# Guilucand/PanDelos

Hardware: AMD Instinct MI355X
Metric: scored gene-pairs/sec (whole node) (higher is better)
Workload: dtype u32 accumulate + f32 finalize

## Files before the change

pandelos_amd/csrc/pdl_api.hip:

```cpp
#include "pdl_common.h"

#include <algorithm>
#include <cstdlib>
#include <cstring>
#include <limits>

static thread_local std::string g_create_error = "";

#define PDL_GUARD_BEGIN try {
#define PDL_GUARD_END(ctx_)                                                       \
    } catch (const pdl_error &e) {                                                \
        if (ctx_) (ctx_)->err = e.msg; else g_create_error = e.msg;               \
        return e.code;                                                            \
    } catch (const std::bad_alloc &) {                                            \
        if (ctx_) (ctx_)->err = "host allocation failed";                         \
        return PDL_ERR_DEVICE;                                                    \
    }

template <class T> static T *xalloc(size_t n) {
    T *p = static_cast<T *>(malloc((n ? n : 1) * sizeof(T)));
    if (!p) throw std::bad_alloc();
    return p;
}

// ... 580 lines not shown
    else if (n == "join_tiny_tier2") c->opt_tiny_tier2 = value != 0;
    else if (n == "join_grid_pct") c->opt_grid_pct = (int) value;
    else if (n == "stage_timers") c->opt_stage_timers = value != 0;
    else if (n == "host_mirror") c->opt_host_mirror = value != 0;
    else if (n == "staging_cap") c->opt_staging_cap = value > 0 ? (uint64_t) value : 0;
    else if (n == "aside_test_reload") c->opt_aside_test_reload = value != 0;
    else if (n == "onepass_scan") c->opt_onepass_scan = value != 0;
    else if (n == "low_memory") c->opt_low_memory = value != 0;
    else if (n == "query_batch_bytes") {
        if (value <= 0) { c->err = "query_batch_bytes: a positive byte count"; return PDL_ERR_ARGUMENT; }
        c->opt_query_batch_bytes = (uint64_t) value;
        return PDL_OK;
    }
    else { c->err = "unknown option " + n; return PDL_ERR_ARGUMENT; }
    c->scored = false;
    return PDL_OK;
}

int pdl_dist_preprocess_begin(pdl_ctx *c, const uint8_t *d_residues, const uint64_t *d_offsets, const uint32_t *d_genome_of,
                              uint32_t n, uint64_t n_res, int k, uint32_t world, uint32_t rank, pdl_dist_slice *out) {
    if (!c || !out) return PDL_ERR_ARGUMENT;
    std::lock_guard<std::mutex> lk(c->mu);
    PDL_GUARD_BEGIN
    if (!d_offsets || !d_genome_of || (!d_residues && n_res)) PDL_FAIL(PDL_ERR_ARGUMENT, "null input pointer");
    if (((uintptr_t) d_residues & 15) != 0) PDL_FAIL(PDL_ERR_ARGUMENT, "d_residues must be 16-byte aligned");
    if (world == 0 || rank >= world || world > 64) PDL_FAIL(PDL_ERR_ARGUMENT, "rank %u of %u (at most 64 ranks)", rank, world);
    PDL_HIP(hipSetDevice(c->device));
    c->preprocessed = false; c->scored = false; c->tasks_ready = false; c->mirror_valid = false;
    c->dist = false; c->dist_stage = 0;
    adopt_device_input(c, d_residues, d_offsets, d_genome_of, n, n_res);
// ... 284 lines not shown
```

pandelos_amd/csrc/pdl_common.h:

```cpp
#pragma once

#include <atomic>
#include <chrono>

#include <hip/hip_runtime.h>

#include <cstdint>
#include <cstdio>
#include <mutex>
#include <cstdlib>
#include <string>
#include <utility>
#include <vector>

#include "../../include/pandelos_amd.h"

#define PDL_WAVE 64

#ifdef __HIPCC__
__device__ __forceinline__ void pdl_sync() {
#ifndef PDL_PLAIN_SYNCTHREADS
    asm volatile("s_waitcnt lgkmcnt(0)" ::: "memory");
#endif
    __syncthreads();
// ... 55 lines not shown
    PDL_JC_ERRORS = 6,
    PDL_JC_CURSOR_T3 = 7,
    PDL_JC_WIDE_ROWS = 9,
    PDL_JC_RELOADS = 10,
    PDL_JC_CURSOR_T0 = 11,
    PDL_JC_ROWS_T0B = 12,
    PDL_JC_CURSOR_T0B = 13,
    PDL_JC_ROWS_T1 = 14,
    PDL_JC_WORDS = 16,
};
enum : uint32_t {
    PDL_JT_CTR_WORDS = 8,
    PDL_JT_EMITTED = 8,
    PDL_JT_RELOADS = PDL_JC_RELOADS,
    PDL_JT_ROWS_T1 = 11,
    PDL_JT_WORDS = 12,
};
static_assert(PDL_JC_ROWS_T1 < PDL_JC_WORDS && PDL_JC_RELOADS < PDL_JT_WORDS && PDL_JC_CURSOR_T3 + 1 == PDL_JT_CTR_WORDS, "join counter layout");

struct pdl_error {
    int code;
    std::string msg;
};

#define PDL_HIP(expr)                                                                           \
    do {                                                                                        \
        hipError_t _e = (expr);                                                                 \
        if (_e != hipSuccess) {                                                                 \
            throw pdl_error{PDL_ERR_DEVICE, std::string(#expr) + ": " + hipGetErrorString(_e)}; \
        }                                                                                       \
    } while (0)
// ... 160 lines not shown
    DevBuf overflow_rows;
    DevBuf gene_info;
    DevBuf join_defer;
    DevBuf glb_table;
    bool glb_clean = false;
    DevBuf row_desc2;
    DevBuf mirror_cnt, mirror_ref;
    DevView taskpos_of;
    std::vector<uint32_t> h_fin;
    bool tasks_ready = false;
    DevBuf scratch2;
    DevBuf task_off;
    int cus = 0;
    uint32_t occ_tier1[5] = {0, 0, 0, 0, 0};
    uint32_t occ_tier0[2] = {0, 0}, occ_tier0b[2] = {0, 0};

    bool edges_valid = false;
    DevBuf bbh_kind, bbh_tab, e_src, e_dst, e_score;
    uint8_t *edge_mirror = nullptr;
    size_t edge_mirror_bytes = 0;
    uint64_t n_edges = 0, n_edges1 = 0;
    std::vector<uint32_t> h_bbh_at;
    std::vector<uint64_t> h_edge1, h_edge_off;

    int opt_tier1 = -1;
    int opt_tier0 = -1;
    int opt_sift_threshold = 1;
    bool opt_tiny_tier2 = false;
    bool opt_stage_timers = true;
    int opt_grid_pct = 0;
// ... 256 lines not shown
```

pandelos_amd/csrc/pdl_join.hip:

```cpp
#include "pdl_common.h"
#include "pdl_scan.h"

#include <algorithm>
#include <cstdlib>
#include <cstring>

constexpr int HBM_THREADS = 512;
constexpr uint32_t EMPTY_KEY = 0xffffffffu;
constexpr uint64_t FIELD_MASK = (1ull << 21) - 1;
constexpr uint32_t CELL_CHUNK = 16384;

struct JoinArgs {
    const uint2 *post;
    const uint4 *ranges;
    const uint2 *ranges8;
    const uint32_t *seq_off;
    const uint32_t *kseq_len;
    const uint32_t *genome_of;
    const uint4 *gene_info;
    const uint32_t *task_rows;
    const uint32_t *task_lg;
    const uint32_t *work;
    const uint4 *desc;
    uint32_t n_work;
// ... 1095 lines not shown
    desc[p] = make_uint4(p, r, e0, seq_off[r + 1] - e0);
}

struct RowCntFlag {
    const uint32_t *row_cnt; const uint32_t *mirror_cnt;
    __device__ uint32_t operator()(uint64_t p) const { return row_cnt[p] + (mirror_cnt ? mirror_cnt[p] : 0u); }
};
struct MirrorCntFlag {
    const uint32_t *mirror_cnt;
    __device__ uint32_t operator()(uint64_t p) const { return mirror_cnt[p]; }
};
struct FinOffApply {
    uint32_t *fin_off;
    __device__ void operator()(uint64_t p, uint32_t, uint32_t prefix) const { fin_off[p] = prefix; }
};
__global__ void k_gather_u32(const uint32_t *src, const uint32_t *idx, uint32_t n, uint32_t *dst, const uint32_t *ctr, const uint32_t *z64) {
    uint32_t i = blockIdx.x * blockDim.x + threadIdx.x;
    if (i < n) dst[i] = src[idx[i]];
    else if (i < n + PDL_JT_CTR_WORDS) dst[i] = ctr[i - n];
    else if (i < n + PDL_JT_EMITTED + 2) dst[i] = z64[i - n - PDL_JT_EMITTED];
    else if (i == n + PDL_JT_RELOADS) dst[i] = ctr[PDL_JC_RELOADS];
    else if (i == n + PDL_JT_ROWS_T1) dst[i] = ctr[PDL_JC_ROWS_T1];
}

struct ZeroRanges { uint4 *p[4]; unsigned long long n16[4]; };
__global__ __launch_bounds__(256) void k_zero_ranges(ZeroRanges z) {
    const unsigned long long stride = (unsigned long long) gridDim.x * 256;
#pragma unroll
    for (int r = 0; r < 4; r++)
        for (unsigned long long i = (unsigned long long) blockIdx.x * 256 + threadIdx.x; i < z.n16[r]; i += stride) z.p[r][i] = make_uint4(0, 0, 0, 0);
}

void pdl_prepare_tasks(pdl_ctx *c) {
    hipStream_t st = c->stream;
    const uint32_t N = c->N, G = c->G;
    if (!c->shard_set) { c->shard.resize(G); for (uint32_t g = 0; g < G; g++) c->shard[g] = g; }
    const uint32_t S = (uint32_t) c->shard.size();
    c->h_local_genome.assign(G, -1);
    c->h_task_row_off.assign(S + 1, 0);
    uint32_t n_rows = 0;
    for (uint32_t i = 0; i < S; i++) n_rows += c->h_genome_row_off[c->shard[i] + 1] - c->h_genome_row_off[c->shard[i]];
    const size_t words = 2 * (size_t) n_rows + N + G;
    const size_t words_all = words + S + 1;
    if (c->task_pin_words < words_all) {
// ... 109 lines not shown
    const size_t hbm_bytes = (size_t) pl.grid3 * N * ((pl.wide ? 2 : 1) * sizeof(uint64_t) + 3 * sizeof(uint32_t));
    if (c->glb_table.bytes < hbm_bytes) { c->glb_table.alloc(hbm_bytes); c->glb_clean = false; }
    if (!c->glb_clean) {
        PDL_HIP(hipMemsetAsync(c->glb_table.p, 0, hbm_bytes, c->stream));
        c->glb_clean = true;
    }
    pl.slack = 2ull * (pl.grid0 + pl.grid0b + pl.grid1 + pl.grid2 + pl.grid3) * CELL_CHUNK;
    return pl;
}

static void score_alloc_rows(pdl_ctx *c, const ScorePlan &pl) {
    const uint32_t N = c->N, G = c->G, n_rows = c->n_task_rows;
    const uint32_t S = (uint32_t) c->shard.size();
    c->MS.alloc((size_t) n_rows * G * sizeof(float) + 16);
    c->CM.alloc((size_t) S * N * sizeof(float) + 16);
    c->row_base.alloc((size_t) n_rows * 4); c->row_cnt.alloc((size_t) n_rows * 4); c->fin_off.alloc(((size_t) n_rows + 2) * 4);
    c->join_ctr.alloc(PDL_JC_WORDS * sizeof(uint32_t));
    c->row_desc.alloc((size_t) n_rows * sizeof(uint4));
    c->row_desc2.alloc((size_t) n_rows * sizeof(uint4) * (pl.tier0 ? 3 : 1));
    c->overflow_rows.alloc((size_t) n_rows * 4 * 4);
    if (pl.mirror) c->mirror_cnt.alloc((size_t) n_rows * 4 * 3 + 16);
    c->gene_info.alloc((size_t) N * sizeof(uint4));
    hipLaunchKernelGGL(k_row_desc, dim3((std::max(n_rows, N) + 255) / 256), dim3(256), 0, c->stream, c->task_rows.as<uint32_t>(), c->seq_off.as<uint32_t>(),
                       n_rows, c->row_desc.as<uint4>(), c->kseq_len.as<uint32_t>(), c->d_gen, c->taskpos_of.as<uint32_t>(), c->local_genome.as<uint32_t>(),
                       N, c->gene_info.as<uint4>());
}

static void score_alloc_cells(pdl_ctx *c, const ScorePlan &pl, unsigned long long cap, unsigned long long extra) {
    const unsigned long long fcap = pl.mirror ? 2 * cap + extra : cap;
    if (fcap >= 0xffffffffull) PDL_FAIL(PDL_ERR_UNSUPPORTED, "more than 2^32 emitted cells on one device: shard the genomes over more devices");
    DevBuf *st[5] = {&c->st_score, &c->st_perc, &c->st_tr, &c->st_col, &c->st_first};
// ... 11 lines not shown
    a.N = c->N; a.G = c->G; a.k = c->rp.k;
    a.min_kseq = (uint32_t) std::max<uint64_t>(c->min_kseq, 1); a.canonical = (c->flags & PDL_FLAG_CANONICAL_ORDER) ? 1u : 0u;
    a.MS = c->MS.as<float>(); a.CM = c->CM.as<float>();
    a.row_base = c->row_base.as<uint32_t>(); a.row_cnt = c->row_cnt.as<uint32_t>();
    a.st_score = c->st_score.as<float>(); a.st_perc = c->st_perc.as<float>(); a.st_tr = c->st_tr.as<float>();
    a.st_col = c->st_col.as<uint32_t>(); a.st_first = c->st_first.as<uint32_t>(); a.st_cap = c->st_cap;
    a.mirror = pl.mirror ? 1u : 0u;
    a.sift_threshold = c->opt_sift_threshold ? 1u : 0u;
    if (pl.mirror) {
        a.taskpos_of = c->taskpos_of.as<uint32_t>(); a.local_genome = c->local_genome.as<uint32_t>();
        a.mirror_cnt = c->mirror_cnt.as<uint32_t>();
    }
    return a;
}

static void score_join(pdl_ctx *c, const ScorePlan &pl) {
    hipStream_t st = c->stream;
    const uint32_t N = c->N, G = c->G, n_rows = c->n_task_rows;
    const uint32_t S = (uint32_t) c->shard.size();
    const int tier1 = pl.tier1;
    {
        auto n16 = [](size_t bytes) { return (unsigned long long) ((bytes + 15) / 16); };
        ZeroRanges z{};
        z.p[0] = c->MS.as<uint4>(); z.n16[0] = n16((size_t) n_rows * G * sizeof(float));
        z.p[1] = c->CM.as<uint4>(); z.n16[1] = n16((size_t) S * N * sizeof(float));
        z.p[2] = c->join_ctr.as<uint4>(); z.n16[2] = n16(PDL_JC_WORDS * sizeof(uint32_t));
        z.p[3] = pl.mirror ? c->mirror_cnt.as<uint4>() : nullptr; z.n16[3] = pl.mirror ? n16((size_t) n_rows * 4 * 3) : 0;
        const unsigned long long most = std::max(z.n16[0], z.n16[1]);
        hipLaunchKernelGGL(k_zero_ranges, dim3((uint32_t) std::min<unsigned long long>((most + 255) / 256 + 1, (unsigned long long) c->cus * 16)), dim3(256), 0, st, z);
    }
    JoinArgs a = join_args(c, pl);
    uint32_t *ctr32 = c->join_ctr.as<uint32_t>();
    uint32_t *list_a = c->overflow_rows.as<uint32_t>(), *list_b = list_a + n_rows, *list_s = list_b + n_rows, *list_s2 = list_s + n_rows;
    a.error_count = ctr32 + PDL_JC_ERRORS; a.reload_count = ctr32 + PDL_JC_RELOADS;
    a.cell_cursor = reinterpret_cast<unsigned long long *>(ctr32 + PDL_JC_CELLS);

    ev_begin(c, EV_JOIN);
    if (pl.wide) {
        hipLaunchKernelGGL(k_iota_u32, dim3((n_rows + 255) / 256), dim3(256), 0, st, list_b, n_rows);
        PDL_HIP(hipMemcpyAsync(ctr32 + PDL_JC_ROWS_T3, &c->n_task_rows, 4, hipMemcpyHostToDevice, st));
    }
    a.work = nullptr; a.desc = c->row_desc.as<uint4>(); a.n_work = pl.wide ? 0 : n_rows; a.n_work_ptr = nullptr;
    if (pl.tier0) {
        a.work_cursor = ctr32 + PDL_JC_CURSOR_T0; a.overflow_count = ctr32 + PDL_JC_ROWS_T0B; a.overflow_rows = list_s; a.work_batch = PT_BATCH;
        a.overflow_desc = c->row_desc2.as<uint4>() + n_rows;
#ifdef PDL_JOIN_PHASES
        static unsigned long long *d_phase0 = nullptr;
        if (!d_phase0) PDL_HIP(hipMalloc((void **) &d_phase0, 12 * sizeof(unsigned long long)));
        PDL_HIP(hipMemsetAsync(d_phase0, 0, 12 * sizeof(unsigned long long), st));
        a.phase = d_phase0;
#endif
        if (pl.tier0_cnt) hipLaunchKernelGGL((k_join_part<PT_T, PT_WG_PER_CU, true>), dim3(pl.grid0), dim3(PT_T), 0, st, a);
        else hipLaunchKernelGGL((k_join_part<PT_T, PT_WG_PER_CU, false>), dim3(pl.grid0), dim3(PT_T), 0, st, a);
#ifdef PDL_JOIN_PHASES
        {
            unsigned long long h[12];
            PDL_HIP(hipMemcpyAsync(h, d_phase0, sizeof(h), hipMemcpyDeviceToHost, st));
            PDL_HIP(hipStreamSynchronize(st));
            const double per = 10.0 / 1000.0 / std::max<uint32_t>(pl.grid0, 1);
            fprintf(stderr, "tier 0 phases per workgroup (us): draw + pick %.1f  stage %.1f  prefixes %.1f  walk %.1f  sift + add %.1f  finalize %.1f  | rows/wg %.1f\n",
                    h[0] * per, h[1] * per, h[2] * per, h[3] * per, h[4] * per, h[5] * per, (double) n_rows / std::max<uint32_t>(pl.grid0, 1));
            fprintf(stderr, "tier 0 counts: cycles %llu (%.2f rows, %.0f lookups each)  cycles that overflowed %llu  survivors of wave 0 %llu (x4 = %.1f %% of the lookups)  probe steps of thread 0: %llu\n",
                    h[6], (double) h[11] / std::max<unsigned long long>(h[6], 1), (double) h[10] / std::max<unsigned long long>(h[6], 1), h[7], h[8], 400.0 * h[8] / std::max<unsigned long long>(h[10], 1), h[9]);
            a.phase = nullptr;
        }
#endif
        a.desc = c->row_desc2.as<uint4>() + n_rows; a.n_work = 0; a.n_work_ptr = ctr32 + PDL_JC_ROWS_T0B;
        a.work_cursor = ctr32 + PDL_JC_CURSOR_T0B; a.overflow_count = ctr32 + PDL_JC_ROWS_T1; a.overflow_rows = list_s2; a.work_batch = 1;
        a.overflow_desc = c->row_desc2.as<uint4>() + 2 * (size_t) n_rows;
        if (pl.tier0_cnt) hipLaunchKernelGGL((k_join_part<PT_T2, PT_WGS2, true>), dim3(pl.grid0b), dim3(PT_T2), 0, st, a);
        else hipLaunchKernelGGL((k_join_part<PT_T2, PT_WGS2, false>), dim3(pl.grid0b), dim3(PT_T2), 0, st, a);
        a.desc = c->row_desc2.as<uint4>() + 2 * (size_t) n_rows; a.n_work = 0; a.n_work_ptr = ctr32 + PDL_JC_ROWS_T1;
        c->tm.join_launches += 2;
    }
    a.work_cursor = ctr32 + PDL_JC_CURSOR_T1; a.overflow_count = ctr32 + PDL_JC_ROWS_T2; a.overflow_rows = list_a; a.overflow_desc = tier1 ? c->row_desc2.as<uint4>() : nullptr;
    a.work_batch = pl.tier0 ? 1 : std::max<uint32_t>(1, std::min<uint32_t>(8, n_rows / (std::max<uint32_t>(pl.grid1, 1) * 8)));
    if (tier1 >= 9 && tier1 <= 11) {
        const unsigned long long avg = n_rows ? c->P / n_rows : 0;
        a.defer_cap = (uint32_t) std::min<unsigned long long>(std::min<unsigned long long>(std::max<unsigned long long>(4 * avg, 8192), 1u << 18), (unsigned long long) N + 64);
        a.defer_wide = (N >= (1u << 22) || pl.wide_aside) ? 1u : 0u;
        c->join_defer.alloc((size_t) pl.grid1 * a.defer_cap * (a.defer_wide ? sizeof(uint4) : sizeof(uint2)));
        a.defer = c->join_defer.p;
        static std::atomic<uint32_t> launch_serial{0};
        a.defer_serial = ++launch_serial;
    }
#ifdef PDL_JOIN_PHASES
    static unsigned long long *d_phase = nullptr;
    if (!d_phase) PDL_HIP(hipMalloc((void **) &d_phase, 10 * sizeof(unsigned long long)));
    PDL_HIP(hipMemsetAsync(d_phase, 0, 10 * sizeof(unsigned long long), st));
// ... 27 lines not shown
    a.hbm_u32 = reinterpret_cast<uint32_t *>(a.hbm_acc + (size_t) pl.grid3 * N * (pl.wide ? 2 : 1));
    a.work = list_b; a.n_work = 0; a.n_work_ptr = ctr32 + PDL_JC_ROWS_T3; a.work_cursor = ctr32 + PDL_JC_CURSOR_T3; a.work_batch = 1;
    ev_begin(c, EV_JOIN_OVF);
    c->glb_clean = false;
    if (pl.wide) hipLaunchKernelGGL(k_join_hbm<true>, dim3(pl.grid3), dim3(HBM_THREADS), 0, st, a);
    else hipLaunchKernelGGL(k_join_hbm<false>, dim3(pl.grid3), dim3(HBM_THREADS), 0, st, a);
    PDL_HIP(hipGetLastError());
    ev_end(c, EV_JOIN_OVF);
    ev_end(c, EV_JOIN);
    c->tm.join_launches += 3;
}

struct JoinCounters {
    uint32_t rows_tier2, rows_tier3, reloads;
    unsigned long long cells;
};
static JoinCounters join_counters(const uint32_t *w) {
    if (w[PDL_JC_ERRORS]) PDL_FAIL(PDL_ERR_DEVICE, "join: %u internal consistency violations", w[PDL_JC_ERRORS]);
    JoinCounters j{w[PDL_JC_ROWS_T2], w[PDL_JC_ROWS_T3], w[PDL_JC_RELOADS], 0};
    memcpy(&j.cells, w + PDL_JC_CELLS, sizeof(j.cells));
    return j;
}

static unsigned long long score_order(pdl_ctx *c, const ScorePlan &pl, const pdl_dist_cell *d_inbox, uint32_t n_inbox, int ev_total) {
    hipStream_t st = c->stream;
    const uint32_t n_rows = c->n_task_rows;
    const uint32_t S = (uint32_t) c->shard.size();
    uint64_t *d_scal = c->scalars.as<uint64_t>();
    uint32_t *ctr32 = c->join_ctr.as<uint32_t>();
    ev_begin(c, EV_ORDER);
    const uint32_t *d_mcnt = pl.mirror ? c->mirror_cnt.as<uint32_t>() : nullptr;
    scan_and_apply(c, n_rows, RowCntFlag{c->row_cnt.as<uint32_t>(), d_mcnt}, FinOffApply{c->fin_off.as<uint32_t>()}, d_scal + PDL_CTL_EMITTED,
                   reinterpret_cast<uint64_t *>(c->fin_off.as<uint32_t>() + n_rows));
    OrderArgs o{};
    if (pl.mirror) {
        uint32_t *m_off = c->mirror_cnt.as<uint32_t>() + n_rows, *m_cur = m_off + n_rows;
        scan_and_apply(c, n_rows, MirrorCntFlag{d_mcnt}, FinOffApply{m_off}, d_scal + PDL_CTL_MIRRORED);
        MirrorArgs ma{};
        ma.row_base = c->row_base.as<uint32_t>(); ma.row_cnt = c->row_cnt.as<uint32_t>(); ma.task_rows = c->task_rows.as<uint32_t>();
        ma.st_score = c->st_score.as<float>(); ma.st_perc = c->st_perc.as<float>(); ma.st_tr = c->st_tr.as<float>();
        ma.st_col = c->st_col.as<uint32_t>(); ma.st_first = c->st_first.as<uint32_t>();
        ma.taskpos_of = c->taskpos_of.as<uint32_t>(); ma.mirror_off = m_off; ma.mirror_cur = m_cur; ma.n_rows = n_rows;
        ma.mcell = c->mirror_ref.as<MCell>();
        hipLaunchKernelGGL(k_mirror_cells, dim3((n_rows + 3) / 4), dim3(256), 0, st, ma);
        if (n_inbox) hipLaunchKernelGGL(k_mirror_cells_inbox, dim3((n_inbox + 255) / 256), dim3(256), 0, st, ma, d_inbox, n_inbox, c->N);
        o.mirror_cnt = d_mcnt; o.mirror_off = m_off; o.mcell = c->mirror_ref.as<MCell>();
    }
    o.row_base = c->row_base.as<uint32_t>(); o.row_cnt = c->row_cnt.as<uint32_t>(); o.fin_off = c->fin_off.as<uint32_t>();
    o.task_rows = c->task_rows.as<uint32_t>();
    o.st_score = c->st_score.as<float>(); o.st_perc = c->st_perc.as<float>(); o.st_tr = c->st_tr.as<float>();
    o.st_col = c->st_col.as<uint32_t>(); o.st_first = c->st_first.as<uint32_t>();
    o.c_score = c->c_score.as<float>(); o.c_perc = c->c_perc.as<float>(); o.c_tr = c->c_tr.as<float>();
    o.c_row = c->c_row.as<int32_t>(); o.c_col = c->c_col.as<int32_t>();
    o.n_rows = n_rows; o.canonical = (c->flags & PDL_FLAG_CANONICAL_ORDER) ? 1u : 0u; o.pack_ok = c->N < (1u << 22) ? 1u : 0u;
    o.wide_rows = ctr32 + PDL_JC_WIDE_ROWS;
    hipLaunchKernelGGL(k_order_rows_wave, dim3((n_rows + 3) / 4), dim3(256), 0, st, o);
    hipLaunchKernelGGL(k_order_rows, dim3(std::min<uint32_t>(n_rows, (uint32_t) c->cus * 8)), dim3(ORDER_THREADS), 0, st, o);
    PDL_HIP(hipGetLastError());
    ev_end(c, EV_ORDER);

    uint32_t *d_idx = c->task_off.as<uint32_t>();
    uint32_t *d_out = d_idx + (S + 1);
    hipLaunchKernelGGL(k_gather_u32, dim3((S + 1 + PDL_JT_WORDS + 255) / 256), dim3(256), 0, st, c->fin_off.as<uint32_t>(), d_idx, S + 1, d_out,
                       ctr32, reinterpret_cast<const uint32_t *>(d_scal + PDL_CTL_EMITTED));
    c->h_fin.resize(S + 1);
    JoinCounters jc;
    uint64_t zsum = 0;
    {
        PinRead rd(c);
        const uint32_t *pf = rd.add<uint32_t>(d_out, S + 1 + PDL_JT_WORDS);
        const uint32_t *lbe = lookback_error_word(c, rd);
        ev_end(c, ev_total);
        rd.sync();
        lookback_check(c, lbe);
        memcpy(c->h_fin.data(), pf, (size_t) (S + 1) * 4);
        const uint32_t *tail = pf + S + 1;
        memcpy(&zsum, tail + PDL_JT_EMITTED, sizeof(zsum));
        c->tm.tier1_rows = pl.tier0 ? tail[PDL_JT_ROWS_T1] : (pl.tier1 ? n_rows : 0);
        c->glb_clean = true;
        jc = join_counters(tail);
    }
    c->tm.aside_reloads = jc.reloads;
    c->tm.overflow_rows = jc.rows_tier3;
    c->tm.tier2_rows = pl.tier1 ? jc.rows_tier2 : n_rows;
    if (jc.cells <= c->st_cap) {
        c->Z = zsum;
        c->tm.emitted_cells = c->Z;
        for (uint32_t i = 0; i <= S; i++) c->h_cell_off[i] = c->h_fin[i];
    }
    return jc.cells;
}

static bool aside_pass_is_suspect(pdl_ctx *c, const ScorePlan &pl) {
    if (pl.wide_aside || c->N >= (1u << 22) || pl.wide || !(pl.tier1 >= 9 && pl.tier1 <= 11)) return false;
    const bool seen = c->tm.aside_reloads != 0 || c->opt_aside_test_reload;
    c->opt_aside_test_reload = false;
    return seen;
}

enum class PassVerdict { accept, repeat_wide_aside, repeat_with_cap };
static PassVerdict judge_pass(pdl_ctx *c, ScorePlan &pl, unsigned long long z, unsigned long long &cap, int attempt, int &overflows) {
    if (aside_pass_is_suspect(c, pl)) {
        if (attempt > 3) PDL_FAIL(PDL_ERR_DEVICE, "put-aside list: reloads persisted");
        pl.wide_aside = true; c->tm.aside_repeats++;
        return PassVerdict::repeat_wide_aside;
// ... 18 lines not shown
    c->tm.scored_lookups = 0; c->tm.walked_lookups = 0; c->tm.outbox_cells = c->tm.inbox_cells = 0;
    c->tm.dist_score_begin_ms = c->tm.dist_score_finish_ms = 0.f;
    if (c->costs_ready) for (uint32_t i = 0; i < S; i++) c->tm.scored_lookups += c->h_genome_cost[c->shard[i]];
    else c->tm.scored_lookups = c->P;
}

void pdl_run_score_all(pdl_ctx *c) {
    ev_begin(c, EV_SCORE_TOTAL);
    if (!c->tasks_ready) pdl_prepare_tasks(c);
    score_reset(c);
    if (c->n_task_rows == 0) { c->scored = true; ev_end(c, EV_SCORE_TOTAL); return; }
    ScorePlan pl = score_plan(c);
    c->tm.walked_lookups = pl.mirror ? (c->P - c->Ushared) / 2 : c->tm.scored_lookups;
    score_alloc_rows(c, pl);
    unsigned long long cap = first_staging_cap(c, pl, c->P);
    for (int attempt = 0, overflows = 0;; attempt++) {
        score_alloc_cells(c, pl, cap, 0);
        score_join(c, pl);
        const unsigned long long z = score_order(c, pl, nullptr, 0, EV_SCORE_TOTAL);
        if (judge_pass(c, pl, z, cap, attempt, overflows) == PassVerdict::accept) break;
        ev_begin(c, EV_SCORE_TOTAL);
    }
    c->tm.join_ms = ev_ms(c, EV_JOIN);
    c->tm.join_overflow_ms = ev_ms(c, EV_JOIN_OVF);
    c->tm.order_ms = ev_ms(c, EV_ORDER);
    c->tm.score_total_ms = ev_ms(c, EV_SCORE_TOTAL);
    c->scored = true;
}

void pdl_run_dist_score_begin(pdl_ctx *c) {
    hipStream_t st = c->stream;
    ev_begin(c, EV_SCORE_TOTAL);
    if (!c->tasks_ready) pdl_prepare_tasks(c);
    score_reset(c);
    const uint32_t W = c->world, n_rows = c->n_task_rows;
    if (W > PDL_MAX_WORLD) PDL_FAIL(PDL_ERR_UNSUPPORTED, "more than %u ranks", PDL_MAX_WORLD);
    c->h_outbox_counts.assign(W, 0);
    c->st_local = 0; c->n_inbox = 0;
    uint64_t upper = 0;
    for (uint32_t g : c->shard) upper += c->h_upper_cost[g];
// ... 65 lines not shown
        ev_end(c, EV_DIST_SCORE_FINISH); c->scored = true; c->dist_stage = 4; return;
    }
    const ScorePlan pl = score_plan(c);
    const unsigned long long cap = c->st_cap;
    if (n_inbox > cap) score_alloc_cells(c, pl, cap, n_inbox);
    else if (2 * cap + n_inbox >= 0xffffffffull) PDL_FAIL(PDL_ERR_UNSUPPORTED, "more than 2^32 emitted cells on one device");
    if (n_inbox) {
        InboxArgs ia{};
        ia.in = d_inbox; ia.n = (uint32_t) n_inbox;
        ia.taskpos_of = c->taskpos_of.as<uint32_t>(); ia.genome_of = c->d_gen; ia.local_genome = c->local_genome.as<uint32_t>();
        ia.mirror_cnt = c->mirror_cnt.as<uint32_t>(); ia.MS = c->MS.as<float>(); ia.CM = c->CM.as<float>();
        ia.N = c->N; ia.G = c->G; ia.error_count = c->join_ctr.as<uint32_t>() + PDL_JC_ERRORS;
        hipLaunchKernelGGL(k_inbox_file, dim3((uint32_t) ((n_inbox + 255) / 256)), dim3(256), 0, st, ia);
        PDL_HIP(hipGetLastError());
    }
    const unsigned long long z = score_order(c, pl, d_inbox, (uint32_t) n_inbox, EV_DIST_SCORE_FINISH);
    if (z > cap) PDL_FAIL(PDL_ERR_DEVICE, "staging cursor moved after the join (%llu > %llu)", z, cap);
    c->tm.order_ms = ev_ms(c, EV_ORDER);
    c->tm.dist_score_finish_ms = ev_ms(c, EV_DIST_SCORE_FINISH);
    c->tm.score_total_ms = c->tm.dist_score_begin_ms + c->tm.dist_score_finish_ms;
    c->scored = true;
    c->dist_stage = 4;
}

#include "pdl_query.h"
#include "pdl_query_batch.h"
```

pandelos_amd/csrc/pdl_scan.h:

```cpp
#pragma once

#include "pdl_common.h"

#include <type_traits>

template <class T, class = void> struct scan_two_phase : std::false_type {};
template <class T> struct scan_two_phase<T, std::void_t<typename T::Loaded>> : std::true_type {};

constexpr int SCAN_THREADS = 256;
constexpr int SCAN_ITEMS = 8;
constexpr int SCAN_TILE = SCAN_THREADS * SCAN_ITEMS;

__device__ __forceinline__ uint32_t wave_inclusive_scan_u32(uint32_t v) {
    const int lane = threadIdx.x & (PDL_WAVE - 1);
#pragma unroll
    for (int d = 1; d < PDL_WAVE; d <<= 1) {
        uint32_t o = __shfl_up(v, d, PDL_WAVE);
        if (lane >= d) v += o;
    }
    return v;
}

__device__ __forceinline__ uint32_t block_exclusive_scan_u32(uint32_t v, uint32_t *s_wave , uint32_t &total) {
    const int lane = threadIdx.x & (PDL_WAVE - 1);
// ... 308 lines not shown
                           (uint32_t) ((tiles + LB_CHUNK - 1) / LB_CHUNK), d_total, d_total2);
        PDL_HIP(hipGetLastError());
        return;
    }
    c->scan_tmp.alloc((size_t) tiles * sizeof(uint32_t));
    uint32_t *ts = c->scan_tmp.as<uint32_t>();
    hipLaunchKernelGGL((k_scan_tile_sums<FlagF>), dim3(tiles), dim3(SCAN_THREADS), 0, c->stream, flag, n, d_n, ts);
    if (tiles <= SCAN_INLINE_TILES) {
        hipLaunchKernelGGL((k_scan_apply<FlagF, ApplyF, true>), dim3(tiles), dim3(SCAN_THREADS), 0, c->stream, flag, apply, n, d_n, ts, d_total, d_total2);
    } else {
        hipLaunchKernelGGL(k_scan_tile_scan, dim3(1), dim3(1024), 0, c->stream, ts, tiles, d_total, d_total2);
        hipLaunchKernelGGL((k_scan_apply<FlagF, ApplyF, false>), dim3(tiles), dim3(SCAN_THREADS), 0, c->stream, flag, apply, n, d_n, ts, d_total, d_total2);
    }
    PDL_HIP(hipGetLastError());
}
```

Before: 1473 billion.

## Launch late join tiers and wide sorter only when counters show work

Splits the join into a front part (tier0) and optional late tiers. Later tiers and the wide-row sorter launch only when device counters read back after ordering show rows that need them, and a sticky per-context flag remembers whether to launch them up front next time. It also fuses the two prefix scans (row counts and mirror counts) into one paired-u32 scan, and zeroes row_cnt inside the existing zero kernel. The cost removed is idle launches of kernels that do no work on typical inputs. In exchange, a second join plus order pass runs when late rows do exist, and the control flow becomes more complex.

New measurement: 1495 billion, median of 6. +1.5%, better.

```diff
diff --git a/pandelos_amd/csrc/pdl_api.hip b/pandelos_amd/csrc/pdl_api.hip
--- a/pandelos_amd/csrc/pdl_api.hip
+++ b/pandelos_amd/csrc/pdl_api.hip
@@ -618,6 +618,7 @@
     }
     else { c->err = "unknown option " + n; return PDL_ERR_ARGUMENT; }
     c->scored = false;
+    c->late_tiers_up_front = c->wide_sorter_up_front = false;
     return PDL_OK;
 }
 
diff --git a/pandelos_amd/csrc/pdl_common.h b/pandelos_amd/csrc/pdl_common.h
--- a/pandelos_amd/csrc/pdl_common.h
+++ b/pandelos_amd/csrc/pdl_common.h
@@ -93,7 +93,8 @@
     PDL_JT_EMITTED = 8,
     PDL_JT_RELOADS = PDL_JC_RELOADS,
     PDL_JT_ROWS_T1 = 11,
-    PDL_JT_WORDS = 12,
+    PDL_JT_WIDE_ROWS = 12,
+    PDL_JT_WORDS = 13,
 };
 static_assert(PDL_JC_ROWS_T1 < PDL_JC_WORDS && PDL_JC_RELOADS < PDL_JT_WORDS && PDL_JC_CURSOR_T3 + 1 == PDL_JT_CTR_WORDS, "join counter layout");
 
@@ -284,6 +285,7 @@
     int cus = 0;
     uint32_t occ_tier1[5] = {0, 0, 0, 0, 0};
     uint32_t occ_tier0[2] = {0, 0}, occ_tier0b[2] = {0, 0};
+    bool late_tiers_up_front = false, wide_sorter_up_front = false;
 
     bool edges_valid = false;
     DevBuf bbh_kind, bbh_tab, e_src, e_dst, e_score;
diff --git a/pandelos_amd/csrc/pdl_join.hip b/pandelos_amd/csrc/pdl_join.hip
--- a/pandelos_amd/csrc/pdl_join.hip
+++ b/pandelos_amd/csrc/pdl_join.hip
@@ -1133,6 +1133,14 @@
     uint32_t *fin_off;
     __device__ void operator()(uint64_t p, uint32_t, uint32_t prefix) const { fin_off[p] = prefix; }
 };
+struct RowPairFlag {
+    const uint32_t *row_cnt; const uint32_t *mirror_cnt;
+    __device__ uint2 operator()(uint64_t p) const { const uint32_t m = mirror_cnt[p]; return make_uint2(row_cnt[p] + m, m); }
+};
+struct FinOffPairApply {
+    uint32_t *fin_off, *m_off;
+    __device__ void operator()(uint64_t p, uint2, uint2 prefix) const { fin_off[p] = prefix.x; m_off[p] = prefix.y; }
+};
 __global__ void k_gather_u32(const uint32_t *src, const uint32_t *idx, uint32_t n, uint32_t *dst, const uint32_t *ctr, const uint32_t *z64) {
     uint32_t i = blockIdx.x * blockDim.x + threadIdx.x;
     if (i < n) dst[i] = src[idx[i]];
@@ -1140,13 +1148,14 @@
     else if (i < n + PDL_JT_EMITTED + 2) dst[i] = z64[i - n - PDL_JT_EMITTED];
     else if (i == n + PDL_JT_RELOADS) dst[i] = ctr[PDL_JC_RELOADS];
     else if (i == n + PDL_JT_ROWS_T1) dst[i] = ctr[PDL_JC_ROWS_T1];
-}
-
-struct ZeroRanges { uint4 *p[4]; unsigned long long n16[4]; };
+    else if (i == n + PDL_JT_WIDE_ROWS) dst[i] = ctr[PDL_JC_WIDE_ROWS];
+}
+
+struct ZeroRanges { uint4 *p[5]; unsigned long long n16[5]; };
 __global__ __launch_bounds__(256) void k_zero_ranges(ZeroRanges z) {
     const unsigned long long stride = (unsigned long long) gridDim.x * 256;
 #pragma unroll
-    for (int r = 0; r < 4; r++)
+    for (int r = 0; r < 5; r++)
         for (unsigned long long i = (unsigned long long) blockIdx.x * 256 + threadIdx.x; i < z.n16[r]; i += stride) z.p[r][i] = make_uint4(0, 0, 0, 0);
 }
 
@@ -1286,7 +1295,7 @@
     const uint32_t S = (uint32_t) c->shard.size();
     c->MS.alloc((size_t) n_rows * G * sizeof(float) + 16);
     c->CM.alloc((size_t) S * N * sizeof(float) + 16);
-    c->row_base.alloc((size_t) n_rows * 4); c->row_cnt.alloc((size_t) n_rows * 4); c->fin_off.alloc(((size_t) n_rows + 2) * 4);
+    c->row_base.alloc((size_t) n_rows * 4); c->row_cnt.alloc((size_t) n_rows * 4 + 16); c->fin_off.alloc(((size_t) n_rows + 2) * 4);
     c->join_ctr.alloc(PDL_JC_WORDS * sizeof(uint32_t));
     c->row_desc.alloc((size_t) n_rows * sizeof(uint4));
     c->row_desc2.alloc((size_t) n_rows * sizeof(uint4) * (pl.tier0 ? 3 : 1));
@@ -1328,18 +1337,19 @@
     return a;
 }
 
-static void score_join(pdl_ctx *c, const ScorePlan &pl) {
+static void score_join(pdl_ctx *c, const ScorePlan &pl, bool front = true, bool back = true) {
     hipStream_t st = c->stream;
     const uint32_t N = c->N, G = c->G, n_rows = c->n_task_rows;
     const uint32_t S = (uint32_t) c->shard.size();
     const int tier1 = pl.tier1;
-    {
+    if (front) {
         auto n16 = [](size_t bytes) { return (unsigned long long) ((bytes + 15) / 16); };
         ZeroRanges z{};
         z.p[0] = c->MS.as<uint4>(); z.n16[0] = n16((size_t) n_rows * G * sizeof(float));
         z.p[1] = c->CM.as<uint4>(); z.n16[1] = n16((size_t) S * N * sizeof(float));
         z.p[2] = c->join_ctr.as<uint4>(); z.n16[2] = n16(PDL_JC_WORDS * sizeof(uint32_t));
         z.p[3] = pl.mirror ? c->mirror_cnt.as<uint4>() : nullptr; z.n16[3] = pl.mirror ? n16((size_t) n_rows * 4 * 3) : 0;
+        z.p[4] = pl.tier0 ? c->row_cnt.as<uint4>() : nullptr; z.n16[4] = pl.tier0 ? n16((size_t) n_rows * 4) : 0;
         const unsigned long long most = std::max(z.n16[0], z.n16[1]);
         hipLaunchKernelGGL(k_zero_ranges, dim3((uint32_t) std::min<unsigned long long>((most + 255) / 256 + 1, (unsigned long long) c->cus * 16)), dim3(256), 0, st, z);
     }
@@ -1350,12 +1360,12 @@
     a.cell_cursor = reinterpret_cast<unsigned long long *>(ctr32 + PDL_JC_CELLS);
 
     ev_begin(c, EV_JOIN);
-    if (pl.wide) {
+    if (pl.wide && front) {
         hipLaunchKernelGGL(k_iota_u32, dim3((n_rows + 255) / 256), dim3(256), 0, st, list_b, n_rows);
         PDL_HIP(hipMemcpyAsync(ctr32 + PDL_JC_ROWS_T3, &c->n_task_rows, 4, hipMemcpyHostToDevice, st));
     }
     a.work = nullptr; a.desc = c->row_desc.as<uint4>(); a.n_work = pl.wide ? 0 : n_rows; a.n_work_ptr = nullptr;
-    if (pl.tier0) {
+    if (pl.tier0 && front) {
         a.work_cursor = ctr32 + PDL_JC_CURSOR_T0; a.overflow_count = ctr32 + PDL_JC_ROWS_T0B; a.overflow_rows = list_s; a.work_batch = PT_BATCH;
         a.overflow_desc = c->row_desc2.as<uint4>() + n_rows;
 #ifdef PDL_JOIN_PHASES
@@ -1384,9 +1394,11 @@
         a.overflow_desc = c->row_desc2.as<uint4>() + 2 * (size_t) n_rows;
         if (pl.tier0_cnt) hipLaunchKernelGGL((k_join_part<PT_T2, PT_WGS2, true>), dim3(pl.grid0b), dim3(PT_T2), 0, st, a);
         else hipLaunchKernelGGL((k_join_part<PT_T2, PT_WGS2, false>), dim3(pl.grid0b), dim3(PT_T2), 0, st, a);
-        a.desc = c->row_desc2.as<uint4>() + 2 * (size_t) n_rows; a.n_work = 0; a.n_work_ptr = ctr32 + PDL_JC_ROWS_T1;
+        PDL_HIP(hipGetLastError());
         c->tm.join_launches += 2;
     }
+    if (!back) { c->ev[EV_JOIN_OVF].used = false; ev_end(c, EV_JOIN); return; }
+    if (pl.tier0) { a.desc = c->row_desc2.as<uint4>() + 2 * (size_t) n_rows; a.n_work = 0; a.n_work_ptr = ctr32 + PDL_JC_ROWS_T1; }
     a.work_cursor = ctr32 + PDL_JC_CURSOR_T1; a.overflow_count = ctr32 + PDL_JC_ROWS_T2; a.overflow_rows = list_a; a.overflow_desc = tier1 ? c->row_desc2.as<uint4>() : nullptr;
     a.work_batch = pl.tier0 ? 1 : std::max<uint32_t>(1, std::min<uint32_t>(8, n_rows / (std::max<uint32_t>(pl.grid1, 1) * 8)));
     if (tier1 >= 9 && tier1 <= 11) {
@@ -1444,15 +1456,40 @@
 struct JoinCounters {
     uint32_t rows_tier2, rows_tier3, reloads;
     unsigned long long cells;
+    uint32_t rows_tier1, wide_rows;
+    unsigned long long emitted;
 };
-static JoinCounters join_counters(const uint32_t *w) {
+static JoinCounters join_counters(const uint32_t *w, bool tail = false) {
     if (w[PDL_JC_ERRORS]) PDL_FAIL(PDL_ERR_DEVICE, "join: %u internal consistency violations", w[PDL_JC_ERRORS]);
-    JoinCounters j{w[PDL_JC_ROWS_T2], w[PDL_JC_ROWS_T3], w[PDL_JC_RELOADS], 0};
+    JoinCounters j{w[PDL_JC_ROWS_T2], w[PDL_JC_ROWS_T3], w[PDL_JC_RELOADS], 0, 0, 0, 0};
     memcpy(&j.cells, w + PDL_JC_CELLS, sizeof(j.cells));
+    if (tail) {
+        j.rows_tier1 = w[PDL_JT_ROWS_T1]; j.wide_rows = w[PDL_JT_WIDE_ROWS];
+        memcpy(&j.emitted, w + PDL_JT_EMITTED, sizeof(j.emitted));
+    }
     return j;
 }
 
-static unsigned long long score_order(pdl_ctx *c, const ScorePlan &pl, const pdl_dist_cell *d_inbox, uint32_t n_inbox, int ev_total) {
+static OrderArgs order_args(pdl_ctx *c, const ScorePlan &pl) {
+    const uint32_t n_rows = c->n_task_rows;
+    OrderArgs o{};
+    if (pl.mirror) { o.mirror_cnt = c->mirror_cnt.as<uint32_t>(); o.mirror_off = o.mirror_cnt + n_rows; o.mcell = c->mirror_ref.as<MCell>(); }
+    o.row_base = c->row_base.as<uint32_t>(); o.row_cnt = c->row_cnt.as<uint32_t>(); o.fin_off = c->fin_off.as<uint32_t>();
+    o.task_rows = c->task_rows.as<uint32_t>();
+    o.st_score = c->st_score.as<float>(); o.st_perc = c->st_perc.as<float>(); o.st_tr = c->st_tr.as<float>();
+    o.st_col = c->st_col.as<uint32_t>(); o.st_first = c->st_first.as<uint32_t>();
+    o.c_score = c->c_score.as<float>(); o.c_perc = c->c_perc.as<float>(); o.c_tr = c->c_tr.as<float>();
+    o.c_row = c->c_row.as<int32_t>(); o.c_col = c->c_col.as<int32_t>();
+    o.n_rows = n_rows; o.canonical = (c->flags & PDL_FLAG_CANONICAL_ORDER) ? 1u : 0u; o.pack_ok = c->N < (1u << 22) ? 1u : 0u;
+    o.wide_rows = c->join_ctr.as<uint32_t>() + PDL_JC_WIDE_ROWS;
+    return o;
+}
+static void launch_order_rows(pdl_ctx *c, const OrderArgs &o) {
+    hipLaunchKernelGGL(k_order_rows, dim3(std::min<uint32_t>(o.n_rows, (uint32_t) c->cus * 8)), dim3(ORDER_THREADS), 0, c->stream, o);
+}
+
+static JoinCounters score_order(pdl_ctx *c, const ScorePlan &pl, const pdl_dist_cell *d_inbox, uint32_t n_inbox, int ev_total,
+                                bool wide_sorter = true, bool again = false) {
     hipStream_t st = c->stream;
     const uint32_t n_rows = c->n_task_rows;
     const uint32_t S = (uint32_t) c->shard.size();
@@ -1460,12 +1497,12 @@
     uint32_t *ctr32 = c->join_ctr.as<uint32_t>();
     ev_begin(c, EV_ORDER);
     const uint32_t *d_mcnt = pl.mirror ? c->mirror_cnt.as<uint32_t>() : nullptr;
-    scan_and_apply(c, n_rows, RowCntFlag{c->row_cnt.as<uint32_t>(), d_mcnt}, FinOffApply{c->fin_off.as<uint32_t>()}, d_scal + PDL_CTL_EMITTED,
-                   reinterpret_cast<uint64_t *>(c->fin_off.as<uint32_t>() + n_rows));
-    OrderArgs o{};
+    uint64_t *d_close = reinterpret_cast<uint64_t *>(c->fin_off.as<uint32_t>() + n_rows);
     if (pl.mirror) {
         uint32_t *m_off = c->mirror_cnt.as<uint32_t>() + n_rows, *m_cur = m_off + n_rows;
-        scan_and_apply(c, n_rows, MirrorCntFlag{d_mcnt}, FinOffApply{m_off}, d_scal + PDL_CTL_MIRRORED);
+        if (again) PDL_HIP(hipMemsetAsync(m_cur, 0, (size_t) n_rows * 4, st));
+        scan_and_apply2(c, n_rows, RowPairFlag{c->row_cnt.as<uint32_t>(), d_mcnt}, FinOffPairApply{c->fin_off.as<uint32_t>(), m_off},
+                        d_scal + PDL_CTL_EMITTED, d_close, d_scal + PDL_CTL_MIRRORED);
         MirrorArgs ma{};
         ma.row_base = c->row_base.as<uint32_t>(); ma.row_cnt = c->row_cnt.as<uint32_t>(); ma.task_rows = c->task_rows.as<uint32_t>();
         ma.st_score = c->st_score.as<float>(); ma.st_perc = c->st_perc.as<float>(); ma.st_tr = c->st_tr.as<float>();
@@ -1474,18 +1511,12 @@
         ma.mcell = c->mirror_ref.as<MCell>();
         hipLaunchKernelGGL(k_mirror_cells, dim3((n_rows + 3) / 4), dim3(256), 0, st, ma);
         if (n_inbox) hipLaunchKernelGGL(k_mirror_cells_inbox, dim3((n_inbox + 255) / 256), dim3(256), 0, st, ma, d_inbox, n_inbox, c->N);
-        o.mirror_cnt = d_mcnt; o.mirror_off = m_off; o.mcell = c->mirror_ref.as<MCell>();
-    }
-    o.row_base = c->row_base.as<uint32_t>(); o.row_cnt = c->row_cnt.as<uint32_t>(); o.fin_off = c->fin_off.as<uint32_t>();
-    o.task_rows = c->task_rows.as<uint32_t>();
-    o.st_score = c->st_score.as<float>(); o.st_perc = c->st_perc.as<float>(); o.st_tr = c->st_tr.as<float>();
-    o.st_col = c->st_col.as<uint32_t>(); o.st_first = c->st_first.as<uint32_t>();
-    o.c_score = c->c_score.as<float>(); o.c_perc = c->c_perc.as<float>(); o.c_tr = c->c_tr.as<float>();
-    o.c_row = c->c_row.as<int32_t>(); o.c_col = c->c_col.as<int32_t>();
-    o.n_rows = n_rows; o.canonical = (c->flags & PDL_FLAG_CANONICAL_ORDER) ? 1u : 0u; o.pack_ok = c->N < (1u << 22) ? 1u : 0u;
-    o.wide_rows = ctr32 + PDL_JC_WIDE_ROWS;
+    } else {
+        scan_and_apply(c, n_rows, RowCntFlag{c->row_cnt.as<uint32_t>(), nullptr}, FinOffApply{c->fin_off.as<uint32_t>()}, d_scal + PDL_CTL_EMITTED, d_close);
+    }
+    const OrderArgs o = order_args(c, pl);
     hipLaunchKernelGGL(k_order_rows_wave, dim3((n_rows + 3) / 4), dim3(256), 0, st, o);
-    hipLaunchKernelGGL(k_order_rows, dim3(std::min<uint32_t>(n_rows, (uint32_t) c->cus * 8)), dim3(ORDER_THREADS), 0, st, o);
+    if (wide_sorter) launch_order_rows(c, o);
     PDL_HIP(hipGetLastError());
     ev_end(c, EV_ORDER);
 
@@ -1495,7 +1526,6 @@
                        ctr32, reinterpret_cast<const uint32_t *>(d_scal + PDL_CTL_EMITTED));
     c->h_fin.resize(S + 1);
     JoinCounters jc;
-    uint64_t zsum = 0;
     {
         PinRead rd(c);
         const uint32_t *pf = rd.add<uint32_t>(d_out, S + 1 + PDL_JT_WORDS);
@@ -1504,21 +1534,19 @@
         rd.sync();
         lookback_check(c, lbe);
         memcpy(c->h_fin.data(), pf, (size_t) (S + 1) * 4);
-        const uint32_t *tail = pf + S + 1;
-        memcpy(&zsum, tail + PDL_JT_EMITTED, sizeof(zsum));
-        c->tm.tier1_rows = pl.tier0 ? tail[PDL_JT_ROWS_T1] : (pl.tier1 ? n_rows : 0);
         c->glb_clean = true;
-        jc = join_counters(tail);
+        jc = join_counters(pf + S + 1, true);
+        c->tm.tier1_rows = pl.tier0 ? jc.rows_tier1 : (pl.tier1 ? n_rows : 0);
     }
     c->tm.aside_reloads = jc.reloads;
     c->tm.overflow_rows = jc.rows_tier3;
     c->tm.tier2_rows = pl.tier1 ? jc.rows_tier2 : n_rows;
     if (jc.cells <= c->st_cap) {
-        c->Z = zsum;
+        c->Z = jc.emitted;
         c->tm.emitted_cells = c->Z;
         for (uint32_t i = 0; i <= S; i++) c->h_cell_off[i] = c->h_fin[i];
     }
-    return jc.cells;
+    return jc;
 }
 
 static bool aside_pass_is_suspect(pdl_ctx *c, const ScorePlan &pl) {
@@ -1567,16 +1595,39 @@
     c->tm.walked_lookups = pl.mirror ? (c->P - c->Ushared) / 2 : c->tm.scored_lookups;
     score_alloc_rows(c, pl);
     unsigned long long cap = first_staging_cap(c, pl, c->P);
+    float join_ms_front = 0.f, order_ms_front = 0.f;
     for (int attempt = 0, overflows = 0;; attempt++) {
         score_alloc_cells(c, pl, cap, 0);
-        score_join(c, pl);
-        const unsigned long long z = score_order(c, pl, nullptr, 0, EV_SCORE_TOTAL);
-        if (judge_pass(c, pl, z, cap, attempt, overflows) == PassVerdict::accept) break;
+        join_ms_front = order_ms_front = 0.f;
+        const bool on_demand = pl.tier0 && !pl.wide && !c->dist;
+        const bool late_tiers = on_demand && !c->late_tiers_up_front, late_sorter = on_demand && !c->wide_sorter_up_front;
+        score_join(c, pl, true, !late_tiers);
+        JoinCounters jc = score_order(c, pl, nullptr, 0, EV_SCORE_TOTAL, !late_sorter, false);
+        if (late_tiers && jc.rows_tier1) {
+            c->late_tiers_up_front = true;
+            join_ms_front = ev_ms(c, EV_JOIN); order_ms_front = ev_ms(c, EV_ORDER);
+            score_join(c, pl, false, true);
+            jc = score_order(c, pl, nullptr, 0, EV_SCORE_TOTAL, true, true);
+            if (jc.wide_rows) c->wide_sorter_up_front = true;
+        } else if (late_sorter && jc.wide_rows) {
+            c->wide_sorter_up_front = true;
+            launch_order_rows(c, order_args(c, pl));
+            PDL_HIP(hipGetLastError());
+            PinRead rd(c);
+            const uint32_t *err = rd.add<uint32_t>(c->join_ctr.as<uint32_t>() + PDL_JC_ERRORS, 1);
+            ev_end(c, EV_SCORE_TOTAL);
+            rd.sync();
+            if (*err) PDL_FAIL(PDL_ERR_DEVICE, "K-order: %u internal consistency violations", *err);
+        } else if (on_demand) {
+            if (!late_tiers && !jc.rows_tier1) c->late_tiers_up_front = false;
+            if (!late_sorter && !jc.wide_rows) c->wide_sorter_up_front = false;
+        }
+        if (judge_pass(c, pl, jc.cells, cap, attempt, overflows) == PassVerdict::accept) break;
         ev_begin(c, EV_SCORE_TOTAL);
     }
-    c->tm.join_ms = ev_ms(c, EV_JOIN);
+    c->tm.join_ms = join_ms_front + ev_ms(c, EV_JOIN);
     c->tm.join_overflow_ms = ev_ms(c, EV_JOIN_OVF);
-    c->tm.order_ms = ev_ms(c, EV_ORDER);
+    c->tm.order_ms = order_ms_front + ev_ms(c, EV_ORDER);
     c->tm.score_total_ms = ev_ms(c, EV_SCORE_TOTAL);
     c->scored = true;
 }
@@ -1672,7 +1723,7 @@
         hipLaunchKernelGGL(k_inbox_file, dim3((uint32_t) ((n_inbox + 255) / 256)), dim3(256), 0, st, ia);
         PDL_HIP(hipGetLastError());
     }
-    const unsigned long long z = score_order(c, pl, d_inbox, (uint32_t) n_inbox, EV_DIST_SCORE_FINISH);
+    const unsigned long long z = score_order(c, pl, d_inbox, (uint32_t) n_inbox, EV_DIST_SCORE_FINISH).cells;
     if (z > cap) PDL_FAIL(PDL_ERR_DEVICE, "staging cursor moved after the join (%llu > %llu)", z, cap);
     c->tm.order_ms = ev_ms(c, EV_ORDER);
     c->tm.dist_score_finish_ms = ev_ms(c, EV_DIST_SCORE_FINISH);
diff --git a/pandelos_amd/csrc/pdl_scan.h b/pandelos_amd/csrc/pdl_scan.h
--- a/pandelos_amd/csrc/pdl_scan.h
+++ b/pandelos_amd/csrc/pdl_scan.h
@@ -346,3 +346,138 @@
     }
     PDL_HIP(hipGetLastError());
 }
+
+__device__ __forceinline__ uint2 block_exclusive_scan_2xu32(uint2 v, uint32_t *s_wave , uint2 &total) {
+    const int lane = threadIdx.x & (PDL_WAVE - 1);
+    const int wave = threadIdx.x / PDL_WAVE;
+    const int nw = blockDim.x / PDL_WAVE;
+    const uint32_t incx = wave_inclusive_scan_u32(v.x), incy = wave_inclusive_scan_u32(v.y);
+    if (lane == PDL_WAVE - 1) { s_wave[wave] = incx; s_wave[17 + wave] = incy; }
+    pdl_sync();
+    if (threadIdx.x == 0) {
+        uint32_t rx = 0, ry = 0;
+        for (int w = 0; w < nw; w++) {
+            const uint32_t tx = s_wave[w], ty = s_wave[17 + w];
+            s_wave[w] = rx; s_wave[17 + w] = ry;
+            rx += tx; ry += ty;
+        }
+        s_wave[16] = rx; s_wave[33] = ry;
+    }
+    pdl_sync();
+    const uint2 res = make_uint2(incx - v.x + s_wave[wave], incy - v.y + s_wave[17 + wave]);
+    total = make_uint2(s_wave[16], s_wave[33]);
+    pdl_sync();
+    return res;
+}
+__device__ __forceinline__ void scan2_store_totals(uint2 all, uint64_t *d_total_x, uint64_t *d_total_x2, uint64_t *d_total_y) {
+    *d_total_x = all.x;
+    *d_total_y = all.y;
+    if (d_total_x2) { reinterpret_cast<uint32_t *>(d_total_x2)[0] = all.x; reinterpret_cast<uint32_t *>(d_total_x2)[1] = 0u; }
+}
+
+template <class FlagF2>
+__global__ __launch_bounds__(SCAN_THREADS) void k_scan2_tile_sums(FlagF2 flag, uint64_t n, uint2 *tile_sums) {
+    __shared__ uint32_t s_wave[34];
+    const uint64_t base = (uint64_t) blockIdx.x * SCAN_TILE;
+    uint2 sum = make_uint2(0u, 0u);
+#pragma unroll
+    for (int j = 0; j < SCAN_ITEMS; j++) {
+        const uint64_t i = base + (uint64_t) j * SCAN_THREADS + threadIdx.x;
+        const uint2 f = flag(i < n ? i : n - 1);
+        sum.x += i < n ? f.x : 0u;
+        sum.y += i < n ? f.y : 0u;
+    }
+    uint2 total;
+    (void) block_exclusive_scan_2xu32(sum, s_wave, total);
+    if (threadIdx.x == 0) tile_sums[blockIdx.x] = total;
+}
+
+static __global__ __launch_bounds__(1024) void k_scan2_tile_scan(uint2 *tile_sums, uint32_t n_tiles, uint64_t *d_total_x, uint64_t *d_total_x2, uint64_t *d_total_y) {
+    __shared__ uint32_t s_wave[34];
+    __shared__ uint2 s_carry;
+    if (threadIdx.x == 0) s_carry = make_uint2(0u, 0u);
+    pdl_sync();
+    for (uint32_t base = 0; base < n_tiles; base += 1024) {
+        const uint32_t i = base + threadIdx.x;
+        const uint2 v = i < n_tiles ? tile_sums[i] : make_uint2(0u, 0u);
+        uint2 total;
+        const uint2 ex = block_exclusive_scan_2xu32(v, s_wave, total);
+        const uint2 carry = s_carry;
+        if (i < n_tiles) tile_sums[i] = make_uint2(ex.x + carry.x, ex.y + carry.y);
+        pdl_sync();
+        if (threadIdx.x == 0) s_carry = make_uint2(carry.x + total.x, carry.y + total.y);
+        pdl_sync();
+    }
+    if (threadIdx.x == 0) scan2_store_totals(s_carry, d_total_x, d_total_x2, d_total_y);
+}
+
+template <class FlagF2, class ApplyF2, bool INLINE_PREFIX>
+__global__ __launch_bounds__(SCAN_THREADS) void k_scan2_apply(FlagF2 flag, ApplyF2 apply, uint64_t n, const uint2 *tile_sums,
+                                                             uint64_t *d_total_x, uint64_t *d_total_x2, uint64_t *d_total_y) {
+    __shared__ uint2 s_flags[SCAN_TILE];
+    __shared__ uint2 s_pref[SCAN_TILE];
+    __shared__ uint32_t s_wave[34];
+    const uint64_t base = (uint64_t) blockIdx.x * SCAN_TILE;
+    uint2 tile_prefix = make_uint2(0u, 0u);
+    if constexpr (INLINE_PREFIX) {
+        const uint32_t upto = blockIdx.x == 0 ? gridDim.x : blockIdx.x;
+        uint2 part = make_uint2(0u, 0u);
+        for (uint32_t i = threadIdx.x; i < upto; i += SCAN_THREADS) { const uint2 t = tile_sums[i]; part.x += t.x; part.y += t.y; }
+        uint2 all;
+        (void) block_exclusive_scan_2xu32(part, s_wave, all);
+        if (blockIdx.x == 0) {
+            if (threadIdx.x == 0) scan2_store_totals(all, d_total_x, d_total_x2, d_total_y);
+        } else {
+            tile_prefix = all;
+        }
+    } else {
+        tile_prefix = tile_sums[blockIdx.x];
+    }
+#pragma unroll
+    for (int j = 0; j < SCAN_ITEMS; j++) {
+        const uint32_t li = j * SCAN_THREADS + threadIdx.x;
+        const uint64_t i = base + li;
+        const uint2 f = flag(i < n ? i : n - 1);
+        s_flags[li] = i < n ? f : make_uint2(0u, 0u);
+    }
+    pdl_sync();
+    uint2 f[SCAN_ITEMS];
+    uint2 sum = make_uint2(0u, 0u);
+#pragma unroll
+    for (int j = 0; j < SCAN_ITEMS; j++) { f[j] = s_flags[threadIdx.x * SCAN_ITEMS + j]; sum.x += f[j].x; sum.y += f[j].y; }
+    uint2 total;
+    uint2 prefix = block_exclusive_scan_2xu32(sum, s_wave, total);
+    prefix.x += tile_prefix.x; prefix.y += tile_prefix.y;
+#pragma unroll
+    for (int j = 0; j < SCAN_ITEMS; j++) { s_pref[threadIdx.x * SCAN_ITEMS + j] = prefix; prefix.x += f[j].x; prefix.y += f[j].y; }
+    pdl_sync();
+#pragma unroll
+    for (int j = 0; j < SCAN_ITEMS; j++) {
+        const uint32_t li = j * SCAN_THREADS + threadIdx.x;
+        const uint64_t i = base + li;
+        if (i < n) apply(i, s_flags[li], s_pref[li]);
+    }
+}
+
+template <class FlagF2, class ApplyF2>
+inline void scan_and_apply2(pdl_ctx *c, uint64_t n, FlagF2 flag, ApplyF2 apply, uint64_t *d_total_x, uint64_t *d_total_x2, uint64_t *d_total_y) {
+    if (n == 0) {
+        PDL_HIP(hipMemsetAsync(d_total_x, 0, sizeof(uint64_t), c->stream));
+        PDL_HIP(hipMemsetAsync(d_total_y, 0, sizeof(uint64_t), c->stream));
+        if (d_total_x2) PDL_HIP(hipMemsetAsync(d_total_x2, 0, sizeof(uint64_t), c->stream));
+        return;
+    }
+    const uint64_t tiles64 = (n + SCAN_TILE - 1) / SCAN_TILE;
+    if (tiles64 > 0x7fffffffull) PDL_FAIL(PDL_ERR_UNSUPPORTED, "scan of %llu elements exceeds the grid limit", (unsigned long long) n);
+    const uint32_t tiles = (uint32_t) tiles64;
+    c->scan_tmp.alloc((size_t) tiles * sizeof(uint2));
+    uint2 *ts = c->scan_tmp.as<uint2>();
+    hipLaunchKernelGGL((k_scan2_tile_sums<FlagF2>), dim3(tiles), dim3(SCAN_THREADS), 0, c->stream, flag, n, ts);
+    if (tiles <= SCAN_INLINE_TILES) {
+        hipLaunchKernelGGL((k_scan2_apply<FlagF2, ApplyF2, true>), dim3(tiles), dim3(SCAN_THREADS), 0, c->stream, flag, apply, n, ts, d_total_x, d_total_x2, d_total_y);
+    } else {
+        hipLaunchKernelGGL(k_scan2_tile_scan, dim3(1), dim3(1024), 0, c->stream, ts, tiles, d_total_x, d_total_x2, d_total_y);
+        hipLaunchKernelGGL((k_scan2_apply<FlagF2, ApplyF2, false>), dim3(tiles), dim3(SCAN_THREADS), 0, c->stream, flag, apply, n, ts, d_total_x, d_total_x2, d_total_y);
+    }
+    PDL_HIP(hipGetLastError());
+}
```
